# PeterouZh/CIPS-3D

Hardware: AMD Instinct MI355X
Metric: rendered imgs/sec (G fwd+bwd) (higher is better)
Workload: dtype f32 (dense layers as 3-pass split-operand MFMA with fp32 accumulate: SIREN forward on fp16 hi/lo planes, ~2e-7 rel., sigma in the fp32 class; INR head and all backward GEMMs on bf16 hi/lo planes, ~5e-6 rel. per layer; everything else fp32); 1 GPU; FFHQ r64, 24 SIREN evals/ray (num_steps 24, hierarchical False), batch 32/GPU, G fwd+bwd, all 9 CIPS blocks; global_batch=32, parallelism=dp1, rccl_ranks=0, inr_gemm_mode=bf16x3, launch=hipGraph replay, grad_reduce=none

## Files before the change

### cips3d_amd/_lib.py

```python
import ctypes as C
import os

_HERE = os.path.dirname(os.path.abspath(__file__))
LIB_PATH = os.path.join(_HERE, "lib", "libcips3d_hip.so")

vp = C.c_void_p
i32 = C.c_int
i64 = C.c_longlong
f32 = C.c_float


class SirenWeights(C.Structure):
    _fields_ = [(n, vp) for n in
                ("w0", "b0", "w1", "b1", "ws", "bs", "wc", "bc", "wf", "bf",
                 "g0", "p0", "g1", "p1", "gc", "pc")] + [("box_scale", f32), ("trig_mode", i32)]


class SirenGrads(C.Structure):
    _fields_ = [(n, vp) for n in ("dg0", "dp0", "dg1", "dp1", "dgc", "dpc", "dw0", "db0", "dw1", "db1", "dws", "dbs", "dwc",
                                  "dbc", "dwf", "dbf")]


class RayParams(C.Structure):
    _fields_ = [("xg", vp), ("yg", vp), ("zg", vp), ("cam2world", vp), ("jitter", vp), ("zvals", vp), ("zc", f32), ("H", i32),
# ... 64 lines not shown
    _fields_ = [("w", vp), ("fwd_hi", vp), ("fwd_lo", vp), ("alt_hi", vp), ("alt_lo", vp), ("scale", f32),
                ("O", i32), ("C", i32), ("kh", i32), ("kw", i32), ("alt_kind", i32), ("bank_off", i32 * 4)]


class ConvWgradDesc(C.Structure):
    _fields_ = [("dy_hi", vp), ("dy_lo", vp), ("x_hi", vp), ("x_lo", vp), ("part", vp),
                ("B", i32), ("C", i32), ("H", i32), ("W", i32), ("O", i32), ("kh", i32), ("kw", i32),
                ("stride", i32), ("pad", i32), ("nchunks", i32)]


SIGNATURES = {
    "cips_version": (i32, []),
    "cips_arch": (C.c_char_p, []),
    "cips_rays_fwd": (i32, [vp, vp, vp, f32, vp, vp, vp, vp, vp, i32, i32, i32, i32, vp]),
    "cips_siren_fwd": (i32, [C.POINTER(SirenWeights), vp, vp, vp, i32, i32, vp]),
    "cips_siren_fwd_x3": (i32, [C.POINTER(SirenWeights), vp, vp, vp, i32, i32, vp]),
    "cips_siren_bwd_rows": (i32, [i32, i32]),
    "cips_siren_bwd_x3_chunks": (i32, [i32, i32]),
    "cips_siren_bwd_x3_gpart": (i32, []),
    "cips_siren_bwd_x3_sred": (i32, []),
    "cips_siren_bwd_x3": (i32, [C.POINTER(SirenWeights), vp, vp, vp, vp, vp, i32, i32, vp]),
    "cips_siren_fwd_x3_rays": (i32, [C.POINTER(SirenWeights), C.POINTER(RayParams), vp, vp, vp, i32, vp]),
    "cips_siren_bwd_x3_rays": (i32, [C.POINTER(SirenWeights), C.POINTER(RayParams), vp, vp, vp, vp, i32, vp]),
    "cips_siren_bwd_x3_finalize": (i32, [C.POINTER(SirenWeights), vp, vp, i32, i32, C.POINTER(SirenGrads), vp]),
    "cips_march_fwd_x3": (i32, [C.POINTER(SirenWeights), C.POINTER(RayParams), vp, f32, i32, i32, vp, vp, vp, vp, vp, vp, i32, vp, vp, vp]),
    "cips_siren_bwd_data": (i32, [C.POINTER(SirenWeights)] + [vp] * 14 + [i32, i32, vp]),
    "cips_siren_bwd_data_f32": (i32, [C.POINTER(SirenWeights)] + [vp] * 9 + [i32, i32, vp]),
    "cips_resample_fwd": (i32, [vp, vp, vp, f32, vp, vp, vp, vp, vp, vp, vp, vp, i32, i32, i32, i32, vp, C.POINTER(RayParams), vp]),
    "cips_composite_fwd": (i32, [vp, vp, vp, vp, vp, vp, vp, f32, vp, vp, vp, vp, vp, i32, i32, i32, i32, vp, vp, vp]),
    "cips_composite_bwd": (i32, [vp, vp, vp, vp, vp, vp, vp, f32, vp, vp, vp, vp, vp, vp, i32, i32, i32, i32, vp, vp]),
    "cips_gemm_f32": (i32, [C.POINTER(GemmDesc), vp]),
    "cips_gemm_bf16x3": (i32, [C.POINTER(GemmX3Desc), vp]),
    "cips_gemm_bf16x3_fuses_torgb": (i32, [C.POINTER(GemmX3Desc)]),
    "cips_gemm_bf16x3_takes_addp": (i32, [C.POINTER(GemmX3Desc)]),
    "cips_torgb_finish": (i32, [vp, i32, vp, vp, i64, i32, vp]),
    "cips_equal_linear_scratch": (i64, [i32, i32, i32, i32]),
    "cips_equal_linear": (i32, [i32, vp, vp, vp, f32, f32, vp, vp, i32, i32, i32, vp]),
    "cips_gemm_bf16x3_km": (i32, [C.POINTER(GemmX3Desc), vp]),
    "cips_gemm_bf16x3_km_grouped": (i32, [C.POINTER(GemmX3Desc), i32, vp]),
    "cips_gemm_bf16": (i32, [C.POINTER(GemmX3Desc), vp]),
    "cips_gemm_bf16_fuses_torgb": (i32, [C.POINTER(GemmX3Desc)]),
    "cips_gemm_bf16_takes_addp": (i32, [C.POINTER(GemmX3Desc)]),
    "cips_gemm_bf16_km": (i32, [C.POINTER(GemmX3Desc), vp]),
    "cips_gemm_bf16_km_grouped": (i32, [C.POINTER(GemmX3Desc), i32, vp]),
    "cips_lrelu_bwd_bias_slices": (i32, [i32]),
    "cips_lrelu_bwd_bias": (i32, [vp, vp, vp, vp, i64, i32, f32, f32, vp]),
    "cips_lrelu_bwd_bias_finish": (i32, [vp, vp, i32, i32, i32, vp]),
    "cips_lrelu_bwd_bias_nhwc_tiles": (i32, [i32]),
    "cips_lrelu_bwd_bias_nhwc": (i32, [vp, vp, vp, vp, vp, i32, i32, i32, f32, f32, vp]),
    "cips_conv1x1_smallk": (i32, [vp, vp, vp, i32, i32, i32, i32, vp]),
    "cips_conv1x1_smallk_bwd_data": (i32, [vp, vp, vp, i32, i32, i32, i32, vp]),
    "cips_conv1x1_smallk_bwd_weight_splits": (i32, [i32, i32]),
    "cips_conv1x1_smallk_bwd_weight": (i32, [vp, vp, vp, i32, i32, i32, i32, vp]),
# ... 77 lines not shown
```

### cips3d_amd/csrc/render.hip

```cpp
#include "common.h"
#include "../../include/cips3d_hip.h"
#include "raygen.h"

namespace {

__global__ __launch_bounds__(256) void rays_kernel(const float* __restrict__ xg, const float* __restrict__ yg,
                                                   const float* __restrict__ zg, float zc,
                                                   const float* __restrict__ c2w, const float* __restrict__ jitter,
                                                   float* __restrict__ points, float* __restrict__ zout,
                                                   float* __restrict__ dirs, int B, int H, int W, int S) {
  const long long total = (long long)B * H * W * S;
  const int n = H * W;
  for (long long idx = (long long)blockIdx.x * blockDim.x + threadIdx.x; idx < total;
       idx += (long long)gridDim.x * blockDim.x) {
    const int i = (int)(idx % S);
    const long long rr = idx / S;
    const int ray = (int)(rr % n);
    const int b = (int)(rr / n);
    const int row = ray / W, col = ray % W;
    const float x = xg[col], y = yg[row];
    const float nrm = sqrtf(x * x + y * y + zc * zc);
    const float dx = x / nrm, dy = y / nrm, dz = zc / nrm;
    float z = zg[i];
    float px = dx * z, py = dy * z, pz = dz * z;
// ... 107 lines not shown
    if (denom < 1e-5f) denom = 1.f;
    const float smp = b0 + (u - c0) / denom * (b1 - b0);
    if (!active) continue;
    a.fine_z[ray * S + i] = smp;
    if (a.fine_pts) {
      float* fp = a.fine_pts + (ray * S + i) * 3;
      fp[0] = ox + dx * smp; fp[1] = oy + dy * smp; fp[2] = oz + dz * smp;
    }
    if (a.inds_out) a.inds_out[ray * S + i] = ind;
    if (a.weights_out) a.weights_out[ray * S + i] = ws[i];
  }
  if (a.cdf_out && active)
    for (int j = sub; j < S - 1; j += SEG) a.cdf_out[ray * (S - 1) + j] = cdf[j];
}

struct CompArgs {
  const float *feat_c, *sig_c, *z_c, *feat_f, *sig_f, *z_f, *noise;
  float noise_std;
  float *fea, *depth, *weights, *zsorted;
  int* order;
  const int* order_in;
  const float* dfea;
  float *dfeat_c, *dsig_c, *dfeat_f, *dsig_f;
  long long R;
  int S, E, clamp_mode, flags;
  const unsigned char* clamp_pin;
  unsigned char* clamp_rec;
};

__device__ __forceinline__ bool clamp_pass(const CompArgs& a, float x, long long idx, bool store) {
  bool pass = x > 0.f;
  if (a.clamp_pin) pass = a.clamp_pin[idx] != 0;
  if (a.clamp_rec && store) a.clamp_rec[idx] = pass ? 1 : 0;
  return pass;
}

__device__ __forceinline__ const float* feat_row(const CompArgs& a, long long ray, int i) {
  if (a.feat_f) return (i < a.S) ? a.feat_f + (ray * a.S + i) * 32 : a.feat_c + (ray * a.S + (i - a.S)) * 32;
  return a.feat_c + (ray * a.S + i) * 32;
}

__global__ __launch_bounds__(256) void composite_fwd_kernel(CompArgs a) {
  extern __shared__ __attribute__((aligned(16))) float sm[];
  const int S = a.S, E = a.E;
  const int rays_per_block = blockDim.x / SEG;
  const int lr = threadIdx.x / SEG, sub = threadIdx.x % SEG;
// ... 144 lines not shown
    s += __shfl_xor(s, 4);
    if (sub == 0) { Ts[k] = Tf; al[k] = alpha; ss[k] = s; }
  }
  __syncthreads();
  float Q = 0.f;
  const float s_off = ((a.flags & 1) ? ss[E - 1] : 0.f) + ((a.flags & 2) ? gsum : 0.f);
  for (int k = E - 1; k >= 0; --k) {
    const int i = ord[k];
    const float alpha = al[k], Tk = Ts[k], s = ss[k] - s_off;
    float w = alpha * Tk;
    if ((a.flags & 1) && k == E - 1) w += 1.f - wsum;

    const float dalpha = Tk * (s - Q);
    Q = fmaf(alpha, s, (1.f - alpha + 1e-10f) * Q);
    float* drow;
    float* dsg;
    if (a.feat_f) {
      drow = (i < S) ? a.dfeat_f + (ray * S + i) * 32 : a.dfeat_c + (ray * S + (i - S)) * 32;
      dsg = (i < S) ? a.dsig_f + ray * S + i : a.dsig_c + ray * S + (i - S);
    } else {
      drow = a.dfeat_c + (ray * S + i) * 32;
      dsg = a.dsig_c + ray * S + i;
    }
    if (active) *reinterpret_cast<float4*>(drow + 4 * sub) = make_float4(w * G.x, w * G.y, w * G.z, w * G.w);
    if ((k % SEG) == sub && active) {
      const float delta = (k + 1 < E) ? (zall[k + 1] - zall[k]) : 1e10f;
      const float x = xs[k];
      float dens = clamp_density(x, a.clamp_mode);
      float dgrad = clamp_density_grad(x, a.clamp_mode);
      if (a.clamp_pin && a.clamp_mode == 0) {
        const bool pass = a.clamp_pin[ray * E + k] != 0;
        dens = pass ? x : 0.f;
        dgrad = pass ? 1.f : 0.f;
      }
      *dsg = dalpha * (delta * expf(-delta * dens)) * dgrad;
    }
  }
}

inline int rays_per_block_for(size_t bytes_per_ray) {
  int r = 32;
  while (r > 1 && (size_t)r * bytes_per_ray > 60 * 1024) r >>= 1;
  return r;
}

}

extern "C" int cips_rays_fwd(const float* xg, const float* yg, const float* zg, float zc,
                             const float* cam2world, const float* jitter, float* points, float* z,
                             float* dirs, int B, int H, int W, int S, cips_stream_t stream) {
  if (B <= 0 || H <= 0 || W <= 0 || S <= 1) return (int)hipErrorInvalidValue;
  long long total = (long long)B * H * W * S;
  int blocks = (int)((total + 255) / 256 < 8192 ? (total + 255) / 256 : 8192);
  hipLaunchKernelGGL(rays_kernel, dim3(blocks), dim3(256), 0, (hipStream_t)stream, xg, yg, zg, zc,
                     cam2world, jitter, points, z, dirs, B, H, W, S);
  return CIPS_CHECK_LAUNCH();
}

extern "C" int cips_resample_fwd(const float* sigma, const float* z, const float* noise, float noise_std,
                                 const float* u, const float* origins, const float* dirs, float* fine_z,
// ... 21 lines not shown
                                  const float* noise, float noise_std, float* fea, float* depth,
                                  float* weights, int* order, float* zsorted, int R, int S,
                                  int clamp_mode, int flags, const unsigned char* clamp_in, unsigned char* clamp_out,
                                  cips_stream_t stream) {
  if (R <= 0 || S <= 0) return (int)hipErrorInvalidValue;
  CompArgs a = {};
  a.feat_c = feat_c; a.sig_c = sig_c; a.z_c = z_c; a.feat_f = feat_f; a.sig_f = sig_f; a.z_f = z_f;
  a.noise = noise; a.noise_std = noise_std; a.fea = fea; a.depth = depth; a.weights = weights;
  a.order = order; a.zsorted = zsorted; a.R = R; a.S = S; a.E = feat_f ? 2 * S : S;
  a.clamp_mode = clamp_mode; a.flags = flags;
  a.clamp_pin = clamp_in; a.clamp_rec = clamp_out;
  size_t per_ray = (size_t)4 * a.E * sizeof(float);
  int rpb = rays_per_block_for(per_ray);
  int blocks = (R + rpb - 1) / rpb;
  hipLaunchKernelGGL(composite_fwd_kernel, dim3(blocks), dim3(rpb * SEG), rpb * per_ray, (hipStream_t)stream, a);
  return CIPS_CHECK_LAUNCH();
}

extern "C" int cips_composite_bwd(const float* feat_c, const float* sig_c, const float* z_c,
                                  const float* feat_f, const float* sig_f, const float* z_f,
                                  const float* noise, float noise_std, const int* order, const float* dfea,
                                  float* dfeat_c, float* dsig_c, float* dfeat_f, float* dsig_f, int R, int S,
                                  int clamp_mode, int flags, const unsigned char* clamp_in, cips_stream_t stream) {
  if (R <= 0 || S <= 0 || (!order && feat_f)) return (int)hipErrorInvalidValue;
  CompArgs a = {};
  a.feat_c = feat_c; a.sig_c = sig_c; a.z_c = z_c; a.feat_f = feat_f; a.sig_f = sig_f; a.z_f = z_f;
  a.noise = noise; a.noise_std = noise_std; a.order_in = order; a.dfea = dfea;
  a.dfeat_c = dfeat_c; a.dsig_c = dsig_c; a.dfeat_f = dfeat_f; a.dsig_f = dsig_f;
  a.R = R; a.S = S; a.E = feat_f ? 2 * S : S; a.clamp_mode = clamp_mode; a.flags = flags;
  a.clamp_pin = clamp_in; a.clamp_rec = nullptr;
  size_t per_ray = (size_t)6 * a.E * sizeof(float);
  int rpb = rays_per_block_for(per_ray);
  int blocks = (R + rpb - 1) / rpb;
  hipLaunchKernelGGL(composite_bwd_kernel, dim3(blocks), dim3(rpb * SEG), rpb * per_ray, (hipStream_t)stream, a);
  return CIPS_CHECK_LAUNCH();
}
```

### cips3d_amd/csrc/siren_bwd_x3.hip

```cpp
#include "common.h"
#include "../../include/cips3d_hip.h"
#include "raygen.h"
#include <type_traits>

#ifdef CIPS_X3_PRIO
#define X3_PRIO(p) __builtin_amdgcn_s_setprio(p)
#else
#define X3_PRIO(p)
#endif

namespace {

typedef __bf16 bf16x8 __attribute__((ext_vector_type(8)));
typedef __bf16 bf16x2 __attribute__((ext_vector_type(2)));
typedef float f32x2 __attribute__((ext_vector_type(2)));
typedef short short4v __attribute__((ext_vector_type(4)));
typedef unsigned int u32x4 __attribute__((ext_vector_type(4)));
typedef unsigned char uchar;

constexpr int H = 128, HC = 64, CF = 32;

constexpr int O_W1H = 0, O_W1L = 32768;
constexpr int O_WCH = 65536, O_WCL = 81920;
constexpr int O_WFH = 98304, O_WFL = 102400;
// ... 281 lines not shown
  put(f.l, 0, lds_tr(ab + c + 2048)); put(f.l, 2, lds_tr(ab + c + 2048 + 64));
#pragma unroll
  for (int i = 0; i < 4; ++i) { f.h[i] &= mask; f.l[i] &= mask; }
}
__device__ __forceinline__ f32x16 x2f(f32x16 acc, const Frag& a, const Frag& b) {
  const bf16x8 bh = mk8(b.h[0], b.h[1], b.h[2], b.h[3]);
  acc = __builtin_amdgcn_mfma_f32_32x32x16_bf16(mk8(a.l[0], a.l[1], a.l[2], a.l[3]), bh, acc, 0, 0, 0);
  acc = __builtin_amdgcn_mfma_f32_32x32x16_bf16(mk8(a.h[0], a.h[1], a.h[2], a.h[3]), bh, acc, 0, 0, 0);
  return acc;
}
__device__ __forceinline__ float4 ld4(const float* p) { return *reinterpret_cast<const float4*>(p); }

struct BwdX3Args {
  cips_siren_weights w;
  const float* points;
  const float* dfeat;
  const float* dsigma;
  float* sred;
  float* gpart;
  int B, P, chunk, chunks;
  unsigned long long* prof;
  int dbg;
  RayGen rg;
};
constexpr int GP_G1 = 0, GP_GC = H * H, GP_GF0 = GP_GC + HC * H, GP_GF1 = GP_GF0 + CF * HC, GPART = GP_GF1 + CF * HC;
constexpr int SRED = 4 * 32 * 8 + 8;

__device__ __forceinline__ float pow2_scale_for(float m, int& k) {
  const unsigned u = __float_as_uint(m);
  const int e = (int)((u >> 23) & 0xffu) - 127;
  k = 13 - e;
  if (!(m > 0.f) || e == 128) k = 0;
  k = k > 100 ? 100 : (k < -100 ? -100 : k);
  return __uint_as_float((unsigned)(k + 127) << 23);
}
template <bool PRE = false, bool F16 = false>
__device__ __forceinline__ void stage_weights_x3(uchar* sm, const cips_siren_weights& w, int b) {
  const int tid = threadIdx.x, nt = blockDim.x;
  const float pre = PRE ? CIPS_INV_2PI : 1.f;
  float s1 = 1.f, sc = 1.f, sf = 1.f, i1 = 1.f, ic = 1.f, isf = 1.f;
  if constexpr (F16) {
    float m1 = 0.f, mc = 0.f, mf = 0.f;
    for (int i = tid; i < H * 32; i += nt) {
      const float4 v = *reinterpret_cast<const float4*>(w.w1 + 4 * i);
      m1 = fmaxf(fmaxf(m1, fmaxf(fabsf(v.x), fabsf(v.y))), fmaxf(fabsf(v.z), fabsf(v.w)));
    }
// ... 396 lines not shown

static int x3_chunk(int B, int P) {
  int chunk = 4096;
  while (chunk > 512 && (long long)B * ((P + chunk - 1) / chunk) < 768) chunk >>= 1;
  return chunk;
}
extern "C" int cips_siren_bwd_x3_chunks(int B, int P) {
  const int chunk = x3_chunk(B, P);
  return (P + chunk - 1) / chunk;
}
extern "C" int cips_siren_bwd_x3_gpart(void) { return GPART; }
#ifdef CIPS_TUNING
static unsigned long long* g_prof = nullptr;
extern "C" int cips_siren_bwd_x3_prof(unsigned long long* host_out) {
  if (!g_prof) return (int)hipErrorNotReady;
  return (int)hipMemcpy(host_out, g_prof, 8 * 4 * 16 * 8, hipMemcpyDeviceToHost);
}
#endif
extern "C" int cips_siren_bwd_x3_sred(void) { return SRED; }


static int siren_bwd_x3_launch(const cips_siren_weights* w, const float* points, const cips_ray_params* rays,
                               const float* dfeat, const float* dsigma, float* sred, float* gpart, int B, int P,
                               cips_stream_t stream);

extern "C" int cips_siren_bwd_x3(const cips_siren_weights* w, const float* points, const float* dfeat,
                                 const float* dsigma, float* sred, float* gpart, int B, int P,
                                 cips_stream_t stream) {
  if (!points) return (int)hipErrorInvalidValue;
  return siren_bwd_x3_launch(w, points, nullptr, dfeat, dsigma, sred, gpart, B, P, stream);
}

extern "C" int cips_siren_bwd_x3_rays(const cips_siren_weights* w, const cips_ray_params* rays, const float* dfeat,
                                      const float* dsigma, float* sred, float* gpart, int B, cips_stream_t stream) {
  if (!rays) return (int)hipErrorInvalidValue;
  return siren_bwd_x3_launch(w, nullptr, rays, dfeat, dsigma, sred, gpart, B, rays->W * rays->H * rays->S, stream);
}

static int siren_bwd_x3_launch(const cips_siren_weights* w, const float* points, const cips_ray_params* rays,
                               const float* dfeat, const float* dsigma, float* sred, float* gpart, int B, int P,
                               cips_stream_t stream) {
  if (!w || !dfeat || !dsigma || !sred || !gpart || B <= 0 || P <= 0) return (int)hipErrorInvalidValue;
  BwdX3Args a;
  a.w = *w; a.points = points; a.dfeat = dfeat; a.dsigma = dsigma; a.sred = sred; a.gpart = gpart;
  a.B = B; a.P = P;
  a.rg = RayGen{};
  if (!points) { const int rc = fill_raygen(a.rg, rays); if (rc) return rc; }
  a.dbg = 0; a.prof = nullptr;
#ifdef CIPS_TUNING
  a.dbg = cips_tune_env("CIPS_X3_DBG", 0);
  static unsigned long long* prof = nullptr;
  static int want_prof = -1;
  if (want_prof < 0) {
    want_prof = cips_tune_env("CIPS_X3_PROF", 0) ? 1 : 0;
    if (want_prof && hipMalloc(&prof, 8 * 4 * 16 * 8) != hipSuccess) prof = nullptr;
  }
  a.prof = prof; g_prof = prof;
#endif
  a.chunk = x3_chunk(B, P);
  a.chunks = (P + a.chunk - 1) / a.chunk;
  dim3 grid(a.chunks, B);
  static bool attr4 = false;
  CIPS_PER_DEVICE(attr4, false);
  if (!attr4) {
    hipFuncSetAttribute((const void*)siren_bwd_x4_kernel<false>, hipFuncAttributeMaxDynamicSharedMemorySize, SMEM_BYTES);
    hipFuncSetAttribute((const void*)siren_bwd_x4_kernel<true>, hipFuncAttributeMaxDynamicSharedMemorySize, SMEM_BYTES);
    attr4 = true;
  }
  if (w->trig_mode & 1)
    hipLaunchKernelGGL(siren_bwd_x4_kernel<true>, grid, dim3(256), SMEM_BYTES, (hipStream_t)stream, a);
  else
    hipLaunchKernelGGL(siren_bwd_x4_kernel<false>, grid, dim3(256), SMEM_BYTES, (hipStream_t)stream, a);
  return CIPS_CHECK_LAUNCH();
}

static int siren_fwd_x3_launch(const cips_siren_weights* w, const float* points, const cips_ray_params* rays, float* feat,
                               float* sigma, float* zout, int B, int P, cips_stream_t stream);

extern "C" int cips_siren_fwd_x3(const cips_siren_weights* w, const float* points, float* feat, float* sigma, int B, int P,
                                 cips_stream_t stream) {
  if (!points) return (int)hipErrorInvalidValue;
  return siren_fwd_x3_launch(w, points, nullptr, feat, sigma, nullptr, B, P, stream);
}

extern "C" int cips_siren_fwd_x3_rays(const cips_siren_weights* w, const cips_ray_params* rays, float* feat, float* sigma,
                                      float* zout, int B, cips_stream_t stream) {
  if (!rays) return (int)hipErrorInvalidValue;
  return siren_fwd_x3_launch(w, nullptr, rays, feat, sigma, zout, B, rays->W * rays->H * rays->S, stream);
}

static int siren_fwd_x3_launch(const cips_siren_weights* w, const float* points, const cips_ray_params* rays, float* feat,
                               float* sigma, float* zout, int B, int P, cips_stream_t stream) {
  if (!w || !feat || !sigma || B <= 0 || P <= 0) return (int)hipErrorInvalidValue;
  FwdX3Args a;
  a.w = *w; a.points = points; a.feat = feat; a.sigma = sigma; a.zout = zout; a.B = B; a.P = P;
// ... 89 lines not shown
```

### cips3d_amd/csrc/siren_bwd_x4.inc

```
__device__ __forceinline__ void pinf(float& x) { asm volatile("" : "+v"(x)); }
__device__ __forceinline__ void pinf(float& a, float& b) { asm volatile("" : "+v"(a), "+v"(b)); }
__device__ __forceinline__ void pinf(float& a, float& b, float& c, float& d) { asm volatile("" : "+v"(a), "+v"(b), "+v"(c), "+v"(d)); }
__device__ __forceinline__ void pinu(unsigned& a, unsigned& b) { asm volatile("" : "+v"(a), "+v"(b)); }
__device__ __forceinline__ void pinu(unsigned& a, unsigned& b, unsigned& c, unsigned& d) { asm volatile("" : "+v"(a), "+v"(b), "+v"(c), "+v"(d)); }

template <bool HW> __device__ __forceinline__ float sin_rev(float x) {
  if (HW) return __builtin_amdgcn_sinf(__builtin_amdgcn_fractf(x));
  float s_, c_; sincos_reduced(reduce_2pi(x), &s_, &c_); return s_;
}

template <bool HW>
__global__ __launch_bounds__(256, 1) void siren_bwd_x4_kernel(BwdX3Args a) {
  extern __shared__ __attribute__((aligned(1024))) uchar smem[];
  const int b = blockIdx.y;
  stage_weights_x3<HW>(smem, a.w, b);
  __syncthreads();
  constexpr float TWO_PI = 6.283185307179586f;

  const int lane0 = threadIdx.x & 63, wave = __builtin_amdgcn_readfirstlane(threadIdx.x >> 6);
  const int cstart = blockIdx.x * a.chunk;
  const int cend = min(cstart + a.chunk, a.P);
  const unsigned sbase = (unsigned)(uintptr_t)((__attribute__((address_space(3))) uchar*)smem);

  f32x16 aG1[4], aGc[2], aGf[1], aS[1];
  zero_acc(aG1); zero_acc(aGc); zero_acc(aGf); zero_acc(aS);
  float r_dsg = 0.f;

  float px, py, pz, dsg;
  {
    const int p = cstart + wave * 32 + (lane0 & 31);
    const bool valid = p < cend;
    const long long gp = (long long)b * a.P + (valid ? p : cend - 1);
    if (a.points) { px = a.points[gp * 3 + 0]; py = a.points[gp * 3 + 1]; pz = a.points[gp * 3 + 2]; }
    else gen_point(a.rg, b, valid ? p : cend - 1, px, py, pz);
    dsg = valid ? a.dsigma[gp] : 0.f;
  }

  constexpr int NPRE = 0;
  Act<4> h1n;
  auto l0_groups = [&](auto G0c, auto G1c, float x, float y, float z) __attribute__((always_inline)) {
    constexpr int G0 = decltype(G0c)::value, G1 = decltype(G1c)::value;
    if (G0 >= G1) return;
    int ln = lane0;
    asm volatile("" : "+v"(ln));
    const unsigned sbase_ = (unsigned)(uintptr_t)((__attribute__((address_space(3))) uchar*)smem);
    const unsigned v64 = opaque(sbase_ + O_L0 + 64 * (ln >> 5));
    float4 pn[4];
#pragma unroll
    for (int e = 0; e < 4; ++e) pn[e] = lds_ld4(v64 + 128 * G0 + 16 * e);
#pragma unroll
    for (int grp = G0; grp < G1; ++grp) {
      float4 pk[4];
#pragma unroll
      for (int e = 0; e < 4; ++e) pk[e] = pn[e];
      if (grp + 1 < G1) {
#pragma unroll
        for (int e = 0; e < 4; ++e) pn[e] = lds_ld4(v64 + 128 * (grp + 1) + 16 * e);
// ... 9 lines not shown
      __builtin_amdgcn_sched_barrier(0);
    }
  };
  using IC0 = std::integral_constant<int, 0>; using ICA = std::integral_constant<int, (NPRE + 2) / 3>;
  using ICB = std::integral_constant<int, (2 * NPRE + 2) / 3>; using ICN = std::integral_constant<int, NPRE>;
  using IC16 = std::integral_constant<int, 16>;
  l0_groups(IC0{}, ICN{}, px, py, pz);

  int rnd = -1;
  for (int pbase = cstart; pbase < cend; pbase += 128) {
    ++rnd;
    X3_TS(0)
    int lane = lane0;
    asm volatile("" : "+v"(lane));
    const int l31 = lane & 31, hf = lane >> 5;
    const LaneAddr LA = lane_addr(lane, sbase);
    const int prow = wave * 32 + l31;
    const unsigned c7 = l31 & 7;
    const unsigned m_d1 = c7 < 4 ? ~0u : 0u, m_d2 = c7 == 4 ? ~0u : 0u, m_h2 = c7 == 5 ? ~0u : 0u;
    const unsigned m_dc = c7 == 6 ? ~0u : 0u, m_df = c7 == 7 ? ~0u : 0u;

    float4 df4[4];
    {
      const int p = pbase + prow;
      const bool valid = p < cend;
      const float* dp = a.dfeat + ((long long)b * a.P + (valid ? p : cend - 1)) * CF + 4 * hf;
#pragma unroll
      for (int g = 0; g < 4; ++g) df4[g] = valid ? ld4(dp + 8 * g) : make_float4(0.f, 0.f, 0.f, 0.f);
    }
    if (hf == 0) {
      uint4 ah, al;
      split2(1.f, px, ah.x, al.x); split2(py, pz, ah.y, al.y); split2(1.f, dsg, ah.z, al.z); split2(1.f, 1.f, ah.w, al.w);
      const u32x4 vh = {ah.x, ah.y, ah.z, ah.w}, vl = {al.x, al.y, al.z, al.w};
      *LDS_PTR(u32x4, sbase + O_AUX + prow * 16) = vh;
      *LDS_PTR(u32x4, sbase + O_AUX + 2048 + prow * 16) = vl;
      r_dsg += dsg;
    }

    const float dsg_s = HW ? dsg * CIPS_INV_2PI : dsg;

    f32x16 acc[4];
    zero_acc(acc);
    float cs2[4][16];
    Act<4> h2p;
    float rv[4], sn[4];
    float4 gq, cq;
    auto film2_slot = [&](int q, int g, int j) __attribute__((always_inline)) {
      const float gg[4] = {gq.x, gq.y, gq.z, gq.w}, cc[4] = {cq.x, cq.y, cq.z, cq.w};
      if (HW) {
// ... 215 lines not shown
          pinf(v4[0], v4[1], v4[2], v4[3]); pinf(w4_[0], w4_[1], w4_[2], w4_[3]);
          if (4 * q + g + 1 < 16) {
            gq2 = lds_ld4(LA.v16 + (O_G1 - O_L0) + 32 * (4 * q + g + 1)); wq2 = lds_ld4(LA.v16 + (O_WS - O_L0) + 32 * (4 * q + g + 1));
          }
        } else if (j == 1) {
          split2(v4[0], v4[1], da2p.hi[q][2 * g], da2p.lo[q][2 * g]);
          split2(v4[2], v4[3], da2p.hi[q][2 * g + 1], da2p.lo[q][2 * g + 1]);
          pinu(da2p.hi[q][2 * g], da2p.lo[q][2 * g], da2p.hi[q][2 * g + 1], da2p.lo[q][2 * g + 1]);
        } else {
          split2(w4_[0], w4_[1], dp2p.hi[q][2 * g], dp2p.lo[q][2 * g]);
          split2(w4_[2], w4_[3], dp2p.hi[q][2 * g + 1], dp2p.lo[q][2 * g + 1]);
          pinu(dp2p.hi[q][2 * g], dp2p.lo[q][2 * g], dp2p.hi[q][2 * g + 1], dp2p.lo[q][2 * g + 1]);
        }
      };
      gq2 = lds_ld4(LA.v16 + (O_G1 - O_L0)); wq2 = lds_ld4(LA.v16 + (O_WS - O_L0));
      layer_tr_mm<4, 4, HC, O_WCH, O_WCL - O_WCH>(LA, dpcp, acc, [&](int slot) __attribute__((always_inline)) {
        const int m = slot / 12, j = slot % 12;
        if (m >= 1) dh2_slot(m - 1, j / 3, j % 3);
      });
#pragma unroll
      for (int j = 0; j < 12; ++j) { dh2_slot(3, j / 3, j % 3); __builtin_amdgcn_sched_barrier(0); }

      {
        const int p = pbase + 128 + prow;
        const bool valid = p < cend;
        const long long gp = (long long)b * a.P + (valid ? p : cend - 1);
        if (a.points) { npx = a.points[gp * 3 + 0]; npy = a.points[gp * 3 + 1]; npz = a.points[gp * 3 + 2]; }
        else gen_point(a.rg, b, valid ? p : cend - 1, npx, npy, npz);
        ndsg = valid ? a.dsigma[gp] : 0.f;
      }
      f32x16 acc1[4];
      zero_acc(acc1);
      float4 pq[4];
      float ar[4], s1[4], c1[4], d1[4];
      auto dh1_slot = [&](int q, int g, int j) __attribute__((always_inline)) {
        if (j == 0) {
#pragma unroll
          for (int e = 0; e < 4; ++e) ar[e] = fmaf(pq[e].x, px, fmaf(pq[e].y, py, fmaf(pq[e].z, pz, pq[e].w)));
          pinf(ar[0], ar[1], ar[2], ar[3]);
          if (4 * q + g + 1 < 16) {
#pragma unroll
            for (int e = 0; e < 4; ++e) pq[e] = lds_ld4(LA.v64 + 128 * (4 * q + g + 1) + 16 * e);
          }
        } else if (j == 1) {
          if (HW) {
#pragma unroll
            for (int e = 0; e < 4; ++e) ar[e] = __builtin_amdgcn_fractf(ar[e]);
            s1[0] = __builtin_amdgcn_sinf(ar[0]); s1[1] = __builtin_amdgcn_sinf(ar[1]);
            pinf(ar[0], ar[1], ar[2], ar[3]); pinf(s1[0], s1[1]);
          } else {
#pragma unroll
// ... 169 lines not shown
```

### cips3d_amd/ops.py

```python
import ctypes as C
import math
import os
import weakref

import torch

from . import _lib
from ._lib import (ConvDgradS2Desc, ConvWgradDesc, ConvX3Desc, GemmDesc, GemmX3Desc, GlinJob, ModfcBwdJob, ModfcPrepJob,
                   RayParams, SirenGrads, SirenWeights, check)

LRELU_SLOPE = 0.2


def _p(t):
    return C.c_void_p(t.data_ptr()) if t is not None else None


def _stream():
    return C.c_void_p(torch.cuda.current_stream().cuda_stream)


def _chk(*tensors):
    for t in tensors:
        if t is None:
# ... 107 lines not shown
        setattr(s, n, _p(t[n]))
    s.box_scale = BOX_SCALE
    s.trig_mode = TRIG_MODE
    return s


def _siren_prep(siren):
    if len(siren) != len(_SIREN_NAMES):
        raise TypeError(f"expected the {len(_SIREN_NAMES)} SIREN tensors {_SIREN_NAMES}, got {len(siren)}")
    t = {n: _c(v.detach()) for n, v in zip(_SIREN_NAMES, siren)}
    _chk(*t.values())
    return t


def _split_k(P, target=8):
    for s in range(target, 0, -1):
        if P % s == 0 and (P // s) % 32 == 0:
            return s
    return 1


SIREN_FWD_MODE = os.environ.get("CIPS_SIREN_FWD", "x3")
SIREN_BWD_MODE = os.environ.get("CIPS_SIREN_BWD", "x3")


class SirenFunction(torch.autograd.Function):

    @staticmethod
    def forward(ctx, points, *siren):
        lib = _lib.load()
        t = _siren_prep(siren)
        points = _c(points.detach())
        _chk(points)
        B, P, _ = points.shape
        feat = torch.empty(B, P, 32, device=points.device)
        sigma = torch.empty(B, P, device=points.device)
        sw = _siren_struct(t)
        fwd = lib.cips_siren_fwd_x3 if SIREN_FWD_MODE == "x3" else lib.cips_siren_fwd
        check(fwd(C.byref(sw), _p(points), _p(feat), _p(sigma), B, P, _stream()), "cips_siren_fwd")
        ctx.save_for_backward(points, *t.values())
        return feat, sigma

    @staticmethod
    def backward(ctx, dfeat, dsigma):
        points = ctx.saved_tensors[0]
        t = dict(zip(_SIREN_NAMES, ctx.saved_tensors[1:]))
        B, P, _ = points.shape
        return (None,) + _siren_backward(t, dfeat, dsigma, B, P, points=points)


def _siren_backward(t, dfeat, dsigma, B, P, points=None, rays=None):
    dev = t["w0"].device
    dfeat = _c(dfeat) if dfeat is not None else torch.zeros(B, P, 32, device=dev)
    dsigma = _c(dsigma) if dsigma is not None else torch.zeros(B, P, device=dev)
    if SIREN_BWD_MODE == "x3" or points is None:
        return _siren_backward_fused(t, dfeat, dsigma, B, P, points, rays)
    return _siren_backward_staged(t, dfeat, dsigma, B, P, points, f32=SIREN_BWD_MODE == "staged_f32")


def _siren_backward_fused(t, dfeat, dsigma, B, P, points, rays):
    lib = _lib.load()
    dev = dfeat.device
    sw = _siren_struct(t)
    chunks = lib.cips_siren_bwd_x3_chunks(B, P)
    gw = lib.cips_siren_bwd_x3_gpart()
    sw_ = lib.cips_siren_bwd_x3_sred()
    sred = torch.empty(B * chunks, sw_, device=dev)
    gpart = torch.empty(B * chunks, gw, device=dev)
    if points is not None:
        check(lib.cips_siren_bwd_x3(C.byref(sw), _p(points), _p(dfeat), _p(dsigma), _p(sred), _p(gpart), B, P,
                                    _stream()), "cips_siren_bwd_x3")
    else:
        check(lib.cips_siren_bwd_x3_rays(C.byref(sw), C.byref(rays), _p(dfeat), _p(dsigma), _p(sred), _p(gpart), B,
                                         _stream()), "cips_siren_bwd_x3_rays")
    outs = tuple(torch.empty_like(t[n]) for n in _SIREN_NAMES)
    sg = SirenGrads()
    for n, v in zip(_SIREN_NAMES, outs):
        setattr(sg, "d" + n, _p(v))
    SRr = sred.view(B, chunks, sw_).sum(1) if chunks > 1 else sred
    Gpr = gpart.view(B, chunks, gw).sum(1) if chunks > 1 else gpart
    check(lib.cips_siren_bwd_x3_finalize(C.byref(sw), _p(SRr), _p(Gpr), B, 1, C.byref(sg), _stream()),
          "cips_siren_bwd_x3_finalize")
    return outs


def _siren_backward_staged(t, dfeat, dsigma, B, P, points, f32):
    lib = _lib.load()
    dev = dfeat.device
    sw = _siren_struct(t)
    BP = B * P
    empty = torch.empty if f32 else Planes.empty
    h1, h2, da2 = (empty(BP, 128, device=dev) for _ in range(3))
# ... 306 lines not shown
        check(lib.cips_march_fwd_x3(C.byref(sw), C.byref(rp), _p(noise), float(noise_std), clamp_mode, flags, _p(fea),
                                    _p(depth), None, _p(feat), _p(sigma), _p(z), B, _p(pin), _p(rec), _stream()),
              "cips_march_fwd_x3")
        if rec is not None and CLAMP_REC is not None:
            CLAMP_REC.append(rec.reshape(B * n, S))
        ctx.clamp_mask = pin
        if train:
            ctx.save_for_backward(xg, yg, zg, cam2world, jitter, noise, feat, sigma, z, *t.values())
        ctx.geom = geom
        ctx.mark_non_differentiable(depth)
        return fea, depth

    @staticmethod
    def backward(ctx, dfea, _ddepth):
        lib = _lib.load()
        xg, yg, zg, cam2world, jitter, noise, feat, sigma, z = ctx.saved_tensors[:9]
        t = dict(zip(_SIREN_NAMES, ctx.saved_tensors[9:]))
        B, H, W, S, zc, noise_std, clamp_mode, flags, _ = ctx.geom
        n = H * W
        R = B * n
        dfea = _c(dfea)
        dfeat = torch.empty_like(feat)
        dsig = torch.empty_like(sigma)
        check(lib.cips_composite_bwd(_p(feat), _p(sigma), _p(z), None, None, None, _p(noise), float(noise_std), None,
                                     _p(dfea), _p(dfeat), _p(dsig), None, None, R, S, clamp_mode, flags, _p(ctx.clamp_mask),
                                     _stream()), "cips_composite_bwd")
        _tail_gate_publish(dfea.device)
        rp = _ray_params(xg, yg, zg, zc, cam2world, jitter, H, W, S)
        grads = _siren_backward(t, dfeat, dsig, B, n * S, rays=rp)
        return (None,) * 7 + grads


def modfc_prep(W, s, eps=1e-8):
    lib = _lib.load()
    in_dim, out_dim = W.shape
    B = s.shape[0]
    dev = W.device
    wb = torch.empty(B, in_dim, out_dim, device=dev)
    wbt = torch.empty(B, out_dim, in_dim, device=dev)
    demod = torch.empty(B, out_dim, device=dev)
    check(lib.cips_modfc_prep(_p(W), _p(s), _p(wb), _p(wbt), _p(demod), B, in_dim, out_dim, eps, _stream()),
          "cips_modfc_prep")
    return wb, wbt, demod


def modfc_prep_bwd(W, s, demod, gwb):
    lib = _lib.load()
    in_dim, out_dim = W.shape
    B = s.shape[0]
    dev = W.device
    cbuf = torch.empty(B, out_dim, device=dev)
    dW = torch.empty(in_dim, out_dim, device=dev)
# ... 1057 lines not shown
```

### include/cips3d_hip.h

```cpp
#ifndef CIPS3D_HIP_H
#define CIPS3D_HIP_H

#ifdef __cplusplus
extern "C" {
#endif

typedef void* cips_stream_t;

int cips_version(void);
const char* cips_arch(void);

int cips_rays_fwd(const float* xg, const float* yg, const float* zg, float zc,
                  const float* cam2world, const float* jitter,
                  float* points, float* z, float* dirs,
                  int B, int H, int W, int S, cips_stream_t stream);

typedef struct cips_siren_weights {
  const float* w0;
  const float* b0;
  const float* w1;
  const float* b1;
  const float* ws;
  const float* bs;
  const float* wc;
// ... 33 lines not shown

typedef struct cips_siren_grads {
  float *dg0, *dp0, *dg1, *dp1, *dgc, *dpc;
  float *dw0, *db0, *dw1, *db1, *dws, *dbs, *dwc, *dbc, *dwf, *dbf;
} cips_siren_grads;
int cips_siren_bwd_x3_finalize(const cips_siren_weights* w, const float* sred, const float* gpart, int B, int chunks,
                               const cips_siren_grads* out, cips_stream_t stream);

typedef struct cips_ray_params {
  const float* xg; const float* yg; const float* zg;
  const float* cam2world;
  const float* jitter;
  const float* zvals;
  float zc;
  int H, W, S;
} cips_ray_params;

int cips_siren_fwd_x3_rays(const cips_siren_weights* w, const cips_ray_params* rays, float* feat, float* sigma,
                           float* zout, int B, cips_stream_t stream);

int cips_siren_bwd_x3_rays(const cips_siren_weights* w, const cips_ray_params* rays, const float* dfeat,
                           const float* dsigma, float* sred, float* gpart, int B, cips_stream_t stream);

int cips_march_fwd_x3(const cips_siren_weights* w, const cips_ray_params* rays, const float* noise, float noise_std,
                      int clamp_mode, int flags, float* fea, float* depth, float* weights, float* feat, float* sigma,
                      float* z, int B, const unsigned char* clamp_in, unsigned char* clamp_out, cips_stream_t stream);

int cips_resample_fwd(const float* sigma, const float* z, const float* noise, float noise_std,
                      const float* u, const float* origins, const float* dirs,
                      float* fine_z, float* fine_pts,
                      float* weights_out, float* cdf_out, long long* inds_out,
                      int B, int n, int S, int clamp_mode, const float* cdf_in, const cips_ray_params* rays,
                      cips_stream_t stream);

int cips_composite_fwd(const float* feat_c, const float* sig_c, const float* z_c,
                       const float* feat_f, const float* sig_f, const float* z_f,
                       const float* noise, float noise_std,
                       float* fea, float* depth, float* weights, int* order, float* zsorted,
                       int R, int S, int clamp_mode, int flags, const unsigned char* clamp_in, unsigned char* clamp_out,
                       cips_stream_t stream);

int cips_composite_bwd(const float* feat_c, const float* sig_c, const float* z_c,
                       const float* feat_f, const float* sig_f, const float* z_f,
                       const float* noise, float noise_std, const int* order,
                       const float* dfea,
                       float* dfeat_c, float* dsig_c, float* dfeat_f, float* dsig_f,
                       int R, int S, int clamp_mode, int flags, const unsigned char* clamp_in, cips_stream_t stream);

typedef struct cips_gemm_desc {
  const float* A; const float* B; float* C;
  int M, N, K;
  int lda, ldb, ldc;
  long long strideA, strideB, strideC;
  int batch;
  int a_kmajor;
  int b_nmajor;
  float alpha;
  const float* bias;
  const float* bias_m;
  int act;
  float slope; float act_gain;
  const float* resid;
  float* C2;
  const float* add;
  const float* rgb_g;
  const float* rgb_w;
  float* C_unmasked;
  const float* mask;
} cips_gemm_desc;

// ... 212 lines not shown
```

Baseline: 2019 img/s.

## Skip SIREN backward for sample points with zero compositing gradient

The composite backward now records a per-point liveness mask: a point is live if its compositing weight or its density gradient is nonzero. A new stream-compaction kernel builds a per-batch list of live point indices and a count. The SIREN backward kernel then iterates only over live points, using indirect indexing, so work on points with zero upstream gradient (transmittance underflow, clamped density) is skipped. This adds a compaction launch, a mask buffer and gather-style loads. The grid stays sized for all points, so blocks beyond the live count exit early.

```diff
diff --git a/cips3d_amd/_lib.py b/cips3d_amd/_lib.py
--- a/cips3d_amd/_lib.py
+++ b/cips3d_amd/_lib.py
@@ -110,6 +110,8 @@
     "cips_siren_bwd_x3": (i32, [C.POINTER(SirenWeights), vp, vp, vp, vp, vp, i32, i32, vp]),
     "cips_siren_fwd_x3_rays": (i32, [C.POINTER(SirenWeights), C.POINTER(RayParams), vp, vp, vp, i32, vp]),
     "cips_siren_bwd_x3_rays": (i32, [C.POINTER(SirenWeights), C.POINTER(RayParams), vp, vp, vp, vp, i32, vp]),
+    "cips_siren_bwd_x3_live": (i32, [C.POINTER(SirenWeights), vp, vp, vp, vp, vp, vp, vp, i32, i32, vp]),
+    "cips_siren_bwd_x3_rays_live": (i32, [C.POINTER(SirenWeights), C.POINTER(RayParams), vp, vp, vp, vp, vp, vp, i32, vp]),
     "cips_siren_bwd_x3_finalize": (i32, [C.POINTER(SirenWeights), vp, vp, i32, i32, C.POINTER(SirenGrads), vp]),
     "cips_march_fwd_x3": (i32, [C.POINTER(SirenWeights), C.POINTER(RayParams), vp, f32, i32, i32, vp, vp, vp, vp, vp, vp, i32, vp, vp, vp]),
     "cips_siren_bwd_data": (i32, [C.POINTER(SirenWeights)] + [vp] * 14 + [i32, i32, vp]),
@@ -117,6 +119,8 @@
     "cips_resample_fwd": (i32, [vp, vp, vp, f32, vp, vp, vp, vp, vp, vp, vp, vp, i32, i32, i32, i32, vp, C.POINTER(RayParams), vp]),
     "cips_composite_fwd": (i32, [vp, vp, vp, vp, vp, vp, vp, f32, vp, vp, vp, vp, vp, i32, i32, i32, i32, vp, vp, vp]),
     "cips_composite_bwd": (i32, [vp, vp, vp, vp, vp, vp, vp, f32, vp, vp, vp, vp, vp, vp, i32, i32, i32, i32, vp, vp]),
+    "cips_composite_bwd_live": (i32, [vp, vp, vp, vp, vp, vp, vp, f32, vp, vp, vp, vp, vp, vp, vp, vp, i32, i32, i32, i32, vp, vp]),
+    "cips_live_points": (i32, [vp, i32, i32, vp, vp, vp]),
     "cips_gemm_f32": (i32, [C.POINTER(GemmDesc), vp]),
     "cips_gemm_bf16x3": (i32, [C.POINTER(GemmX3Desc), vp]),
     "cips_gemm_bf16x3_fuses_torgb": (i32, [C.POINTER(GemmX3Desc)]),
diff --git a/cips3d_amd/csrc/render.hip b/cips3d_amd/csrc/render.hip
--- a/cips3d_amd/csrc/render.hip
+++ b/cips3d_amd/csrc/render.hip
@@ -153,6 +153,7 @@
   const int* order_in;
   const float* dfea;
   float *dfeat_c, *dsig_c, *dfeat_f, *dsig_f;
+  unsigned char *live_c, *live_f;
   long long R;
   int S, E, clamp_mode, flags;
   const unsigned char* clamp_pin;
@@ -343,7 +344,8 @@
       drow = a.dfeat_c + (ray * S + i) * 32;
       dsg = a.dsig_c + ray * S + i;
     }
-    if (active) *reinterpret_cast<float4*>(drow + 4 * sub) = make_float4(w * G.x, w * G.y, w * G.z, w * G.w);
+    if (active && !a.live_c) *reinterpret_cast<float4*>(drow + 4 * sub) = make_float4(w * G.x, w * G.y, w * G.z, w * G.w);
+    float dsv = 0.f;
     if ((k % SEG) == sub && active) {
       const float delta = (k + 1 < E) ? (zall[k + 1] - zall[k]) : 1e10f;
       const float x = xs[k];
@@ -354,9 +356,65 @@
         dens = pass ? x : 0.f;
         dgrad = pass ? 1.f : 0.f;
       }
-      *dsg = dalpha * (delta * expf(-delta * dens)) * dgrad;
-    }
-  }
+      dsv = dalpha * (delta * expf(-delta * dens)) * dgrad;
+      *dsg = dsv;
+    }
+    if (a.live_c) {
+      const float dsb = __shfl(dsv, k % SEG, SEG);
+      const bool live = (w != 0.f) || (dsb != 0.f);
+      if (active && live) *reinterpret_cast<float4*>(drow + 4 * sub) = make_float4(w * G.x, w * G.y, w * G.z, w * G.w);
+      unsigned char* lv = a.live_c + ray * S + i;
+      if (a.feat_f) lv = (i < S) ? a.live_f + ray * S + i : a.live_c + ray * S + (i - S);
+      if ((k % SEG) == sub && active) *lv = live ? 1 : 0;
+    }
+  }
+}
+
+constexpr int LIVE_THREADS = 1024, LIVE_TILE = LIVE_THREADS * 16;
+__global__ __launch_bounds__(LIVE_THREADS) void live_points_kernel(const unsigned char* __restrict__ live, int P,
+                                                                   int* __restrict__ idx, int* __restrict__ count) {
+  __shared__ int wsum[LIVE_THREADS / 64];
+  const int b = blockIdx.x, tid = threadIdx.x, lane = tid & 63, wave = tid >> 6;
+  const unsigned char* src = live + (long long)b * P;
+  int* dst = idx + (long long)b * P;
+  const bool vec = (P & 15) == 0 && (reinterpret_cast<uintptr_t>(live) & 15) == 0;
+  auto load16 = [&](int o) {
+    uint4 v = make_uint4(0u, 0u, 0u, 0u);
+    if (o >= P) return v;
+    if (vec) return *reinterpret_cast<const uint4*>(src + o);
+    unsigned wd[4] = {0u, 0u, 0u, 0u};
+    for (int j = 0; j < 16 && o + j < P; ++j) wd[j >> 2] |= (unsigned)src[o + j] << (8 * (j & 3));
+    return make_uint4(wd[0], wd[1], wd[2], wd[3]);
+  };
+  int base = 0;
+  uint4 cur = load16(tid * 16);
+  for (int t0 = 0; t0 < P; t0 += LIVE_TILE) {
+    const int o = t0 + tid * 16;
+    const uint4 nxt = load16(o + LIVE_TILE);
+    const unsigned wd[4] = {cur.x, cur.y, cur.z, cur.w};
+    int n = 0;
+#pragma unroll
+    for (int j = 0; j < 16; ++j) n += ((wd[j >> 2] >> (8 * (j & 3))) & 0xffu) ? 1 : 0;
+    int incl = n;
+#pragma unroll
+    for (int off = 1; off < 64; off <<= 1) {
+      const int u = __shfl_up(incl, off);
+      if (lane >= off) incl += u;
+    }
+    if (lane == 63) wsum[wave] = incl;
+    __syncthreads();
+    int before = 0, total = 0;
+#pragma unroll
+    for (int wv = 0; wv < LIVE_THREADS / 64; ++wv) { const int c = wsum[wv]; before += wv < wave ? c : 0; total += c; }
+    int pos = base + before + incl - n;
+#pragma unroll
+    for (int j = 0; j < 16; ++j)
+      if ((wd[j >> 2] >> (8 * (j & 3))) & 0xffu) dst[pos++] = o + j;
+    base += total;
+    cur = nxt;
+    __syncthreads();
+  }
+  if (tid == 0) count[b] = base;
 }
 
 inline int rays_per_block_for(size_t bytes_per_ray) {
@@ -424,11 +482,29 @@
                                   const float* noise, float noise_std, const int* order, const float* dfea,
                                   float* dfeat_c, float* dsig_c, float* dfeat_f, float* dsig_f, int R, int S,
                                   int clamp_mode, int flags, const unsigned char* clamp_in, cips_stream_t stream) {
+  return cips_composite_bwd_live(feat_c, sig_c, z_c, feat_f, sig_f, z_f, noise, noise_std, order, dfea, dfeat_c, dsig_c,
+                                 dfeat_f, dsig_f, nullptr, nullptr, R, S, clamp_mode, flags, clamp_in, stream);
+}
+
+extern "C" int cips_live_points(const unsigned char* live, int B, int P, int* idx, int* count, cips_stream_t stream) {
+  if (!live || !idx || !count || B <= 0 || P <= 0) return (int)hipErrorInvalidValue;
+  hipLaunchKernelGGL(live_points_kernel, dim3(B), dim3(LIVE_THREADS), 0, (hipStream_t)stream, live, P, idx, count);
+  return CIPS_CHECK_LAUNCH();
+}
+
+extern "C" int cips_composite_bwd_live(const float* feat_c, const float* sig_c, const float* z_c,
+                                       const float* feat_f, const float* sig_f, const float* z_f,
+                                       const float* noise, float noise_std, const int* order, const float* dfea,
+                                       float* dfeat_c, float* dsig_c, float* dfeat_f, float* dsig_f,
+                                       unsigned char* live_c, unsigned char* live_f, int R, int S,
+                                       int clamp_mode, int flags, const unsigned char* clamp_in, cips_stream_t stream) {
   if (R <= 0 || S <= 0 || (!order && feat_f)) return (int)hipErrorInvalidValue;
+  if ((live_c || live_f) && (!live_c || (feat_f && !live_f))) return (int)hipErrorInvalidValue;
   CompArgs a = {};
   a.feat_c = feat_c; a.sig_c = sig_c; a.z_c = z_c; a.feat_f = feat_f; a.sig_f = sig_f; a.z_f = z_f;
   a.noise = noise; a.noise_std = noise_std; a.order_in = order; a.dfea = dfea;
   a.dfeat_c = dfeat_c; a.dsig_c = dsig_c; a.dfeat_f = dfeat_f; a.dsig_f = dsig_f;
+  a.live_c = live_c; a.live_f = live_f;
   a.R = R; a.S = S; a.E = feat_f ? 2 * S : S; a.clamp_mode = clamp_mode; a.flags = flags;
   a.clamp_pin = clamp_in; a.clamp_rec = nullptr;
   size_t per_ray = (size_t)6 * a.E * sizeof(float);
diff --git a/cips3d_amd/csrc/siren_bwd_x3.hip b/cips3d_amd/csrc/siren_bwd_x3.hip
--- a/cips3d_amd/csrc/siren_bwd_x3.hip
+++ b/cips3d_amd/csrc/siren_bwd_x3.hip
@@ -327,6 +327,8 @@
   unsigned long long* prof;
   int dbg;
   RayGen rg;
+  const int* idx;
+  const int* count;
 };
 constexpr int GP_G1 = 0, GP_GC = H * H, GP_GF0 = GP_GC + HC * H, GP_GF1 = GP_GF0 + CF * HC, GPART = GP_GF1 + CF * HC;
 constexpr int SRED = 4 * 32 * 8 + 8;
@@ -769,7 +771,7 @@
 
 static int siren_bwd_x3_launch(const cips_siren_weights* w, const float* points, const cips_ray_params* rays,
                                const float* dfeat, const float* dsigma, float* sred, float* gpart, int B, int P,
-                               cips_stream_t stream);
+                               cips_stream_t stream, const int* idx = nullptr, const int* count = nullptr);
 
 extern "C" int cips_siren_bwd_x3(const cips_siren_weights* w, const float* points, const float* dfeat,
                                  const float* dsigma, float* sred, float* gpart, int B, int P,
@@ -784,11 +786,26 @@
   return siren_bwd_x3_launch(w, nullptr, rays, dfeat, dsigma, sred, gpart, B, rays->W * rays->H * rays->S, stream);
 }
 
+extern "C" int cips_siren_bwd_x3_live(const cips_siren_weights* w, const float* points, const float* dfeat,
+                                      const float* dsigma, const int* idx, const int* count, float* sred, float* gpart,
+                                      int B, int P, cips_stream_t stream) {
+  if (!points || !idx || !count) return (int)hipErrorInvalidValue;
+  return siren_bwd_x3_launch(w, points, nullptr, dfeat, dsigma, sred, gpart, B, P, stream, idx, count);
+}
+
+extern "C" int cips_siren_bwd_x3_rays_live(const cips_siren_weights* w, const cips_ray_params* rays, const float* dfeat,
+                                           const float* dsigma, const int* idx, const int* count, float* sred,
+                                           float* gpart, int B, cips_stream_t stream) {
+  if (!rays || !idx || !count) return (int)hipErrorInvalidValue;
+  return siren_bwd_x3_launch(w, nullptr, rays, dfeat, dsigma, sred, gpart, B, rays->W * rays->H * rays->S, stream, idx, count);
+}
+
 static int siren_bwd_x3_launch(const cips_siren_weights* w, const float* points, const cips_ray_params* rays,
                                const float* dfeat, const float* dsigma, float* sred, float* gpart, int B, int P,
-                               cips_stream_t stream) {
+                               cips_stream_t stream, const int* idx, const int* count) {
   if (!w || !dfeat || !dsigma || !sred || !gpart || B <= 0 || P <= 0) return (int)hipErrorInvalidValue;
   BwdX3Args a;
+  a.idx = idx; a.count = count;
   a.w = *w; a.points = points; a.dfeat = dfeat; a.dsigma = dsigma; a.sred = sred; a.gpart = gpart;
   a.B = B; a.P = P;
   a.rg = RayGen{};
@@ -810,14 +827,20 @@
   static bool attr4 = false;
   CIPS_PER_DEVICE(attr4, false);
   if (!attr4) {
-    hipFuncSetAttribute((const void*)siren_bwd_x4_kernel<false>, hipFuncAttributeMaxDynamicSharedMemorySize, SMEM_BYTES);
-    hipFuncSetAttribute((const void*)siren_bwd_x4_kernel<true>, hipFuncAttributeMaxDynamicSharedMemorySize, SMEM_BYTES);
+    hipFuncSetAttribute((const void*)siren_bwd_x4_kernel<false, false>, hipFuncAttributeMaxDynamicSharedMemorySize, SMEM_BYTES);
+    hipFuncSetAttribute((const void*)siren_bwd_x4_kernel<true, false>, hipFuncAttributeMaxDynamicSharedMemorySize, SMEM_BYTES);
+    hipFuncSetAttribute((const void*)siren_bwd_x4_kernel<false, true>, hipFuncAttributeMaxDynamicSharedMemorySize, SMEM_BYTES);
+    hipFuncSetAttribute((const void*)siren_bwd_x4_kernel<true, true>, hipFuncAttributeMaxDynamicSharedMemorySize, SMEM_BYTES);
     attr4 = true;
   }
-  if (w->trig_mode & 1)
-    hipLaunchKernelGGL(siren_bwd_x4_kernel<true>, grid, dim3(256), SMEM_BYTES, (hipStream_t)stream, a);
-  else
-    hipLaunchKernelGGL(siren_bwd_x4_kernel<false>, grid, dim3(256), SMEM_BYTES, (hipStream_t)stream, a);
+  const bool hw = (w->trig_mode & 1) != 0;
+  if (idx) {
+    if (hw) hipLaunchKernelGGL((siren_bwd_x4_kernel<true, true>), grid, dim3(256), SMEM_BYTES, (hipStream_t)stream, a);
+    else hipLaunchKernelGGL((siren_bwd_x4_kernel<false, true>), grid, dim3(256), SMEM_BYTES, (hipStream_t)stream, a);
+  } else {
+    if (hw) hipLaunchKernelGGL((siren_bwd_x4_kernel<true, false>), grid, dim3(256), SMEM_BYTES, (hipStream_t)stream, a);
+    else hipLaunchKernelGGL((siren_bwd_x4_kernel<false, false>), grid, dim3(256), SMEM_BYTES, (hipStream_t)stream, a);
+  }
   return CIPS_CHECK_LAUNCH();
 }
 
diff --git a/cips3d_amd/csrc/siren_bwd_x4.inc b/cips3d_amd/csrc/siren_bwd_x4.inc
--- a/cips3d_amd/csrc/siren_bwd_x4.inc
+++ b/cips3d_amd/csrc/siren_bwd_x4.inc
@@ -9,7 +9,7 @@
   float s_, c_; sincos_reduced(reduce_2pi(x), &s_, &c_); return s_;
 }
 
-template <bool HW>
+template <bool HW, bool LIVE>
 __global__ __launch_bounds__(256, 1) void siren_bwd_x4_kernel(BwdX3Args a) {
   extern __shared__ __attribute__((aligned(1024))) uchar smem[];
   const int b = blockIdx.y;
@@ -18,8 +18,15 @@
   constexpr float TWO_PI = 6.283185307179586f;
 
   const int lane0 = threadIdx.x & 63, wave = __builtin_amdgcn_readfirstlane(threadIdx.x >> 6);
-  const int cstart = blockIdx.x * a.chunk;
-  const int cend = min(cstart + a.chunk, a.P);
+  int cstart = blockIdx.x * a.chunk;
+  int cend = min(cstart + a.chunk, a.P);
+  if (LIVE) {
+    const int cnt = a.count[b];
+    const int len = ((cnt + a.chunks - 1) / a.chunks + 127) & ~127;
+    cstart = blockIdx.x * len;
+    cend = min(cstart + len, cnt);
+  }
+  const int* const lidx = LIVE ? a.idx + (long long)b * a.P : nullptr;
   const unsigned sbase = (unsigned)(uintptr_t)((__attribute__((address_space(3))) uchar*)smem);
 
   f32x16 aG1[4], aGc[2], aGf[1], aS[1];
@@ -28,11 +35,13 @@
 
   float px, py, pz, dsg;
   {
-    const int p = cstart + wave * 32 + (lane0 & 31);
-    const bool valid = p < cend;
-    const long long gp = (long long)b * a.P + (valid ? p : cend - 1);
+    const int slot = cstart + wave * 32 + (lane0 & 31);
+    const bool valid = slot < cend;
+    int p = valid ? slot : cend - 1;
+    if (LIVE) p = cend > 0 ? lidx[p] : 0;
+    const long long gp = (long long)b * a.P + p;
     if (a.points) { px = a.points[gp * 3 + 0]; py = a.points[gp * 3 + 1]; pz = a.points[gp * 3 + 2]; }
-    else gen_point(a.rg, b, valid ? p : cend - 1, px, py, pz);
+    else gen_point(a.rg, b, p, px, py, pz);
     dsg = valid ? a.dsigma[gp] : 0.f;
   }
 
@@ -88,9 +97,11 @@
 
     float4 df4[4];
     {
-      const int p = pbase + prow;
-      const bool valid = p < cend;
-      const float* dp = a.dfeat + ((long long)b * a.P + (valid ? p : cend - 1)) * CF + 4 * hf;
+      const int slot = pbase + prow;
+      const bool valid = slot < cend;
+      int p = valid ? slot : cend - 1;
+      if (LIVE) p = lidx[p];
+      const float* dp = a.dfeat + ((long long)b * a.P + p) * CF + 4 * hf;
 #pragma unroll
       for (int g = 0; g < 4; ++g) df4[g] = valid ? ld4(dp + 8 * g) : make_float4(0.f, 0.f, 0.f, 0.f);
     }
@@ -352,11 +363,13 @@
       for (int j = 0; j < 12; ++j) { dh2_slot(3, j / 3, j % 3); __builtin_amdgcn_sched_barrier(0); }
 
       {
-        const int p = pbase + 128 + prow;
-        const bool valid = p < cend;
-        const long long gp = (long long)b * a.P + (valid ? p : cend - 1);
+        const int slot = pbase + 128 + prow;
+        const bool valid = slot < cend;
+        int p = valid ? slot : cend - 1;
+        if (LIVE) p = lidx[p];
+        const long long gp = (long long)b * a.P + p;
         if (a.points) { npx = a.points[gp * 3 + 0]; npy = a.points[gp * 3 + 1]; npz = a.points[gp * 3 + 2]; }
-        else gen_point(a.rg, b, valid ? p : cend - 1, npx, npy, npz);
+        else gen_point(a.rg, b, p, npx, npy, npz);
         ndsg = valid ? a.dsigma[gp] : 0.f;
       }
       f32x16 acc1[4];
diff --git a/cips3d_amd/ops.py b/cips3d_amd/ops.py
--- a/cips3d_amd/ops.py
+++ b/cips3d_amd/ops.py
@@ -153,6 +153,7 @@
 
 SIREN_FWD_MODE = os.environ.get("CIPS_SIREN_FWD", "x3")
 SIREN_BWD_MODE = os.environ.get("CIPS_SIREN_BWD", "x3")
+SIREN_BWD_LIVE = os.environ.get("CIPS_SIREN_BWD_LIVE", "1") != "0"
 
 
 class SirenFunction(torch.autograd.Function):
@@ -180,16 +181,26 @@
         return (None,) + _siren_backward(t, dfeat, dsigma, B, P, points=points)
 
 
-def _siren_backward(t, dfeat, dsigma, B, P, points=None, rays=None):
+def _siren_backward(t, dfeat, dsigma, B, P, points=None, rays=None, live=None):
     dev = t["w0"].device
     dfeat = _c(dfeat) if dfeat is not None else torch.zeros(B, P, 32, device=dev)
     dsigma = _c(dsigma) if dsigma is not None else torch.zeros(B, P, device=dev)
     if SIREN_BWD_MODE == "x3" or points is None:
-        return _siren_backward_fused(t, dfeat, dsigma, B, P, points, rays)
+        return _siren_backward_fused(t, dfeat, dsigma, B, P, points, rays, live)
+    assert live is None
     return _siren_backward_staged(t, dfeat, dsigma, B, P, points, f32=SIREN_BWD_MODE == "staged_f32")
 
 
-def _siren_backward_fused(t, dfeat, dsigma, B, P, points, rays):
+def live_points(mask):
+    lib = _lib.load()
+    B, P = mask.shape
+    idx = torch.empty(B, P, dtype=torch.int32, device=mask.device)
+    count = torch.empty(B, dtype=torch.int32, device=mask.device)
+    check(lib.cips_live_points(_p(mask), B, P, _p(idx), _p(count), _stream()), "cips_live_points")
+    return idx, count
+
+
+def _siren_backward_fused(t, dfeat, dsigma, B, P, points, rays, live=None):
     lib = _lib.load()
     dev = dfeat.device
     sw = _siren_struct(t)
@@ -198,7 +209,15 @@
     sw_ = lib.cips_siren_bwd_x3_sred()
     sred = torch.empty(B * chunks, sw_, device=dev)
     gpart = torch.empty(B * chunks, gw, device=dev)
-    if points is not None:
+    if live is not None:
+        idx, count = live
+        if points is not None:
+            check(lib.cips_siren_bwd_x3_live(C.byref(sw), _p(points), _p(dfeat), _p(dsigma), _p(idx), _p(count), _p(sred),
+                                             _p(gpart), B, P, _stream()), "cips_siren_bwd_x3_live")
+        else:
+            check(lib.cips_siren_bwd_x3_rays_live(C.byref(sw), C.byref(rays), _p(dfeat), _p(dsigma), _p(idx), _p(count),
+                                                  _p(sred), _p(gpart), B, _stream()), "cips_siren_bwd_x3_rays_live")
+    elif points is not None:
         check(lib.cips_siren_bwd_x3(C.byref(sw), _p(points), _p(dfeat), _p(dsigma), _p(sred), _p(gpart), B, P,
                                     _stream()), "cips_siren_bwd_x3")
     else:
@@ -551,12 +570,19 @@
         dfea = _c(dfea)
         dfeat = torch.empty_like(feat)
         dsig = torch.empty_like(sigma)
-        check(lib.cips_composite_bwd(_p(feat), _p(sigma), _p(z), None, None, None, _p(noise), float(noise_std), None,
-                                     _p(dfea), _p(dfeat), _p(dsig), None, None, R, S, clamp_mode, flags, _p(ctx.clamp_mask),
-                                     _stream()), "cips_composite_bwd")
+        use_live = SIREN_BWD_LIVE and SIREN_BWD_MODE == "x3"
+        if use_live:
+            mask = torch.empty(B, n * S, dtype=torch.uint8, device=dfea.device)
+            check(lib.cips_composite_bwd_live(_p(feat), _p(sigma), _p(z), None, None, None, _p(noise), float(noise_std), None,
+                                              _p(dfea), _p(dfeat), _p(dsig), None, None, _p(mask), None, R, S, clamp_mode, flags,
+                                              _p(ctx.clamp_mask), _stream()), "cips_composite_bwd_live")
+        else:
+            check(lib.cips_composite_bwd(_p(feat), _p(sigma), _p(z), None, None, None, _p(noise), float(noise_std), None,
+                                         _p(dfea), _p(dfeat), _p(dsig), None, None, R, S, clamp_mode, flags, _p(ctx.clamp_mask),
+                                         _stream()), "cips_composite_bwd")
         _tail_gate_publish(dfea.device)
         rp = _ray_params(xg, yg, zg, zc, cam2world, jitter, H, W, S)
-        grads = _siren_backward(t, dfeat, dsig, B, n * S, rays=rp)
+        grads = _siren_backward(t, dfeat, dsig, B, n * S, rays=rp, live=live_points(mask) if use_live else None)
         return (None,) * 7 + grads
 
 
diff --git a/include/cips3d_hip.h b/include/cips3d_hip.h
--- a/include/cips3d_hip.h
+++ b/include/cips3d_hip.h
@@ -79,6 +79,12 @@
 int cips_siren_bwd_x3_rays(const cips_siren_weights* w, const cips_ray_params* rays, const float* dfeat,
                            const float* dsigma, float* sred, float* gpart, int B, cips_stream_t stream);
 
+int cips_siren_bwd_x3_live(const cips_siren_weights* w, const float* points, const float* dfeat, const float* dsigma,
+                           const int* idx, const int* count, float* sred, float* gpart, int B, int P, cips_stream_t stream);
+int cips_siren_bwd_x3_rays_live(const cips_siren_weights* w, const cips_ray_params* rays, const float* dfeat,
+                                const float* dsigma, const int* idx, const int* count, float* sred, float* gpart, int B,
+                                cips_stream_t stream);
+
 int cips_march_fwd_x3(const cips_siren_weights* w, const cips_ray_params* rays, const float* noise, float noise_std,
                       int clamp_mode, int flags, float* fea, float* depth, float* weights, float* feat, float* sigma,
                       float* z, int B, const unsigned char* clamp_in, unsigned char* clamp_out, cips_stream_t stream);
@@ -103,6 +109,16 @@
                        const float* dfea,
                        float* dfeat_c, float* dsig_c, float* dfeat_f, float* dsig_f,
                        int R, int S, int clamp_mode, int flags, const unsigned char* clamp_in, cips_stream_t stream);
+
+int cips_composite_bwd_live(const float* feat_c, const float* sig_c, const float* z_c,
+                            const float* feat_f, const float* sig_f, const float* z_f,
+                            const float* noise, float noise_std, const int* order,
+                            const float* dfea,
+                            float* dfeat_c, float* dsig_c, float* dfeat_f, float* dsig_f,
+                            unsigned char* live_c, unsigned char* live_f,
+                            int R, int S, int clamp_mode, int flags, const unsigned char* clamp_in, cips_stream_t stream);
+
+int cips_live_points(const unsigned char* live, int B, int P, int* idx, int* count, cips_stream_t stream);
 
 typedef struct cips_gemm_desc {
   const float* A; const float* B; float* C;
```

Result: faster. 2077 img/s, median of 6 (+2.8%).
